# wangzy22/UniPre3D

Measured on AMD Instinct MI355X. Metric: rendered_views_per_sec, higher is better.
Workload: dtype f32; 1 GPU; C2: render-loss hot path (activations + render fwd + loss + render bwd), object-level, P=128 Gaussians/object, 256x256, B=32/GPU x V=4 views = 128 renders/GPU/step; head output o ~ N(0,1) i.i.d. (SURVEY 8d primary regime); global_batch=32, parallelism=dp1, loss=focal_l2, autograd_entry=loss.backward()

## Files before the change

### unipre3d_amd/csrc/u3d_render.hip

```cpp
#include "u3d_common.h"
#ifdef U3D_TIMELINE
#include <cstdio>
#include <vector>
#endif

namespace {

constexpr float LOG2E = 1.4426950408889634f;
constexpr float ALPHA_MIN = 1.0f / 255.0f;
constexpr float T_STOP = 0.0001f;

__device__ __forceinline__ bool rect_hits(const uint2 r, int tx, int ty) {
  const int x0 = r.x & 0xffffu, y0 = r.x >> 16, x1 = r.y & 0xffffu, y1 = r.y >> 16;
  return tx >= x0 && tx < x1 && ty >= y0 && ty < y1;
}

struct LossCtx {
  int kind;
  float w_bg, w_non, b0, b1, b2, t0, t1, t2;
};
__device__ __forceinline__ LossCtx loss_ctx(const U3DLoss& L, const float* __restrict__ bg) {
  const float b0 = bg[0], b1 = bg[1], b2 = bg[2];
  return LossCtx{L.kind, L.w_bg, L.w_non, b0, b1, b2, 1e-6f + 1e-5f * fabsf(b0), 1e-6f + 1e-5f * fabsf(b1), 1e-6f + 1e-5f * fabsf(b2)};
}
// ... 191 lines not shown
        }
      }
#pragma unroll
      for (int k = 0; k < 4; ++k) {
        F.C0[k] = fmaf(Q.z, wv[k], F.C0[k]);
        F.C1[k] = fmaf(Q.w, wv[k], F.C1[k]);
        F.C2[k] = fmaf(R.x, wv[k], F.C2[k]);
        if (DEPTH) F.Dv[k] = fmaf(invd, wv[k], F.Dv[k]);
        F.Tr[k] = tn[k];
      }
      if (contrib != 0ull) { jlast = j; blast = b; }
      if (some_stop) {
#pragma unroll
        for (int k = 0; k < 4; ++k) {
          amin[k] = mask_sel(m_stop[k], 2.f, amin[k]);
          F.stop_pos[k] = __float_as_uint(mask_sel(m_stop[k], R.y, __uint_as_float(F.stop_pos[k])));
        }
        const bool all_done = amin[0] > 1.f && amin[1] > 1.f && amin[2] > 1.f && amin[3] > 1.f;
        if (__ballot(!all_done) == 0ull) { wave_done = true; break; }
      }
    }
    if (blast == b) F.wlast = __builtin_amdgcn_readfirstlane(__float_as_uint(L.P2[jlast].y));
    __builtin_amdgcn_fence(__ATOMIC_RELEASE, "wavefront");
    __builtin_amdgcn_wave_barrier();
  }
  return true;
}

template <typename T>
__device__ __forceinline__ T moment_to_acc(int k, const T* m, float a, float b, float c, float op, float half_w, float half_h) {
  switch (k) {
    case 0: return -(T)half_w * ((T)a * m[0] + (T)b * m[1]);
    case 1: return -(T)half_h * ((T)c * m[1] + (T)b * m[0]);
    case 2: return (T)-0.5 * m[2];
    case 3: return (T)-0.5 * m[3];
    case 4: return (T)-0.5 * m[4];
    case 5: return m[5] != (T)0 ? m[5] / (T)op : (T)0;
    default: return m[k];
  }
}

template <bool HAS_INVD, int PB , bool PLAIN >
__device__ __forceinline__ void tile_backward(const TileLds& L, const TileGeom& G, int lane, uint32_t wmax, int staged,
                                              lanemask_t staged_bal, float pyf, const float (&pxf)[4],
                                              const uint32_t (&lim)[4], float (&Tr)[4], float (&Rk)[4],
                                              const float (&dp0)[4], const float (&dp1)[4], const float (&dp2)[4],
                                              const float (&dinv)[4], float half_w, float half_h, size_t NG,
                                              double* __restrict__ acc, float* __restrict__ pt, uint32_t* __restrict__ pcnt) {
  constexpr int NK = HAS_INVD ? U3D_NACC : U3D_NACC - 1;
  const int bank = (lane >> 2) & 3;
  const bool writer = (lane & 3) == 0 && lane < 16;
  typedef __attribute__((address_space(3))) float lds_float;
  const uint32_t acc_lane = (uint32_t)(uintptr_t)(lds_float*)&L.acc[0][0] + 4u * (uint32_t)bank;
  const int nb = (int)((wmax + U3D_WAVE - 1) / U3D_WAVE);
  for (int b = nb - 1; b >= 0; --b) {
    lanemask_t bal = staged_bal;
    if (b != staged) { bool plain; bal = tile_stage<HAS_INVD>(L, G, lane, b, wmax, plain); staged = b; staged_bal = bal; }
    const uint32_t lm = wmax - (uint32_t)b * U3D_WAVE;
    const int total = lm >= U3D_WAVE ? __popcll(bal) : __popcll(bal & ((1ull << lm) - 1ull));
    for (int j = total - 1; j >= 0; --j) {
      const float4 A = L.P0[j];
      const float4 Q = L.P1[j];
      const float2 R = L.P2[j];
      const float invd = HAS_INVD ? L.D[j] : 0.f;
      const uint32_t pos = __float_as_uint(R.y);
      const float dy = A.y - pyf;
      const float bdy = A.w * dy, cdy2 = (Q.x * dy) * dy;
      float dx[4], ae[4], ar[4];
      lanemask_t any = 0ull;
      if (PLAIN) alpha_run(A.x, A.z, bdy, cdy2, Q.y, L.S[j * L.sstride], pxf[0], ar);
#pragma unroll
      for (int k = 0; k < 4; ++k) {
        dx[k] = A.x - pxf[k];
        float pw = 0.f;
        if (!PLAIN) {
          pw = fmaf(fmaf(A.z, dx[k], bdy), dx[k], cdy2);
          ar[k] = Q.y * __builtin_amdgcn_exp2f(pw);
        }
        const float araw = ar[k];
        const lanemask_t m_a = (PLAIN ? ~0ull : __builtin_amdgcn_fcmpf(pw, 0.f, U3D_FCMP_OLE)) & __builtin_amdgcn_fcmpf(araw, ALPHA_MIN, U3D_FCMP_OGE);
        ae[k] = mask_combine_sel0(m_a, __builtin_amdgcn_uicmp(pos, lim[k], U3D_ICMP_ULT), any, araw);
      }
      if (any == 0ull) continue;
      float m0, mx, mxx, g_r, g_g, g_b, g_d = 0.f;
#pragma unroll
      for (int k = 0; k < 4; ++k) {
        const float alpha = PLAIN ? ae[k] : min_099(ae[k]);
        const float om = 1.f - alpha;
        const float rc = __builtin_amdgcn_rcpf(om);
        const float Tn = Tr[k] * rc;
        const float w = alpha * Tn;
        Tr[k] = Tn;
        float cdp = fmaf(R.x, dp2[k], fmaf(Q.w, dp1[k], Q.z * dp0[k]));
        if (HAS_INVD) cdp = fmaf(invd, dinv[k], cdp);
        const float dL_dalpha = fmaf(Tn, cdp, -(Rk[k] * rc));
        Rk[k] = fmaf(w, cdp, Rk[k]);
        const float q = ae[k] * dL_dalpha;
        const float qdx = q * dx[k];
        if (k == 0) {
          g_r = w * dp0[k]; g_g = w * dp1[k]; g_b = w * dp2[k];
          if (HAS_INVD) g_d = w * dinv[k];
          m0 = q; mx = qdx; mxx = qdx * dx[k];
        } else {
          g_r = fmaf(w, dp0[k], g_r); g_g = fmaf(w, dp1[k], g_g); g_b = fmaf(w, dp2[k], g_b);
          if (HAS_INVD) g_d = fmaf(w, dinv[k], g_d);
          m0 += q; mx += qdx;
          mxx = fmaf(qdx, dx[k], mxx);
        }
      }
      asm volatile("s_nop 1\n\t"
                   "v_add_f32_dpp %0, %0, %0 quad_perm:[1,0,3,2] row_mask:0xf bank_mask:0xf\n\t"
                   "v_add_f32_dpp %1, %1, %1 quad_perm:[1,0,3,2] row_mask:0xf bank_mask:0xf\n\t"
                   "v_add_f32_dpp %2, %2, %2 quad_perm:[1,0,3,2] row_mask:0xf bank_mask:0xf\n\t"
                   "v_add_f32_dpp %3, %3, %3 quad_perm:[1,0,3,2] row_mask:0xf bank_mask:0xf\n\t"
                   "v_add_f32_dpp %4, %4, %4 quad_perm:[1,0,3,2] row_mask:0xf bank_mask:0xf\n\t"
                   "v_add_f32_dpp %5, %5, %5 quad_perm:[1,0,3,2] row_mask:0xf bank_mask:0xf\n\t"
                   "v_add_f32_dpp %0, %0, %0 quad_perm:[2,3,0,1] row_mask:0xf bank_mask:0xf\n\t"
                   "v_add_f32_dpp %1, %1, %1 quad_perm:[2,3,0,1] row_mask:0xf bank_mask:0xf\n\t"
                   "v_add_f32_dpp %2, %2, %2 quad_perm:[2,3,0,1] row_mask:0xf bank_mask:0xf\n\t"
                   "v_add_f32_dpp %3, %3, %3 quad_perm:[2,3,0,1] row_mask:0xf bank_mask:0xf\n\t"
                   "v_add_f32_dpp %4, %4, %4 quad_perm:[2,3,0,1] row_mask:0xf bank_mask:0xf\n\t"
                   "v_add_f32_dpp %5, %5, %5 quad_perm:[2,3,0,1] row_mask:0xf bank_mask:0xf\n\t"
                   "s_nop 1"
                   : "+v"(m0), "+v"(mx), "+v"(mxx), "+v"(g_r), "+v"(g_g), "+v"(g_b));
      if (HAS_INVD)
        asm volatile("s_nop 1\n\t"
                     "v_add_f32_dpp %0, %0, %0 quad_perm:[1,0,3,2] row_mask:0xf bank_mask:0xf\n\t"
                     "s_nop 1\n\t"
                     "v_add_f32_dpp %0, %0, %0 quad_perm:[2,3,0,1] row_mask:0xf bank_mask:0xf\n\t"
                     "s_nop 1"
                     : "+v"(g_d));
      float my = dy * m0, mxy = dy * mx;
      float myy = dy * my;
      if (HAS_INVD)
        asm volatile("s_nop 1\n\t"
                     "v_add_f32_dpp %0, %0, %0 row_half_mirror row_mask:0xf bank_mask:0x5\n\t"
                     "v_add_f32_dpp %1, %1, %1 row_half_mirror row_mask:0xf bank_mask:0x5\n\t"
                     "v_add_f32_dpp %2, %2, %2 row_half_mirror row_mask:0xf bank_mask:0x5\n\t"
                     "v_add_f32_dpp %3, %3, %3 row_half_mirror row_mask:0xf bank_mask:0x5\n\t"
                     "v_add_f32_dpp %4, %4, %4 row_half_mirror row_mask:0xf bank_mask:0x5\n\t"
                     "v_add_f32_dpp %0, %5, %5 row_half_mirror row_mask:0xf bank_mask:0xa\n\t"
                     "v_add_f32_dpp %1, %6, %6 row_half_mirror row_mask:0xf bank_mask:0xa\n\t"
                     "v_add_f32_dpp %2, %7, %7 row_half_mirror row_mask:0xf bank_mask:0xa\n\t"
                     "v_add_f32_dpp %3, %8, %8 row_half_mirror row_mask:0xf bank_mask:0xa\n\t"
                     "v_add_f32_dpp %4, %9, %9 row_half_mirror row_mask:0xf bank_mask:0xa\n\t"
                     "v_add_f32_dpp %0, %0, %0 row_ror:8 row_mask:0xf bank_mask:0x3\n\t"
                     "v_add_f32_dpp %2, %2, %2 row_ror:8 row_mask:0xf bank_mask:0x3\n\t"
                     "v_add_f32_dpp %4, %4, %4 row_ror:8 row_mask:0xf bank_mask:0xf\n\t"
                     "v_add_f32_dpp %0, %1, %1 row_ror:8 row_mask:0xf bank_mask:0xc\n\t"
                     "v_add_f32_dpp %2, %3, %3 row_ror:8 row_mask:0xf bank_mask:0xc\n\t"
                     "s_nop 1"
                     : "+v"(mx), "+v"(mxx), "+v"(myy), "+v"(g_r), "+v"(g_b)
                     : "v"(my), "v"(mxy), "v"(m0), "v"(g_g), "v"(g_d));
      else
        asm volatile("s_nop 1\n\t"
                     "v_add_f32_dpp %0, %0, %0 row_half_mirror row_mask:0xf bank_mask:0x5\n\t"
                     "v_add_f32_dpp %1, %1, %1 row_half_mirror row_mask:0xf bank_mask:0x5\n\t"
                     "v_add_f32_dpp %2, %2, %2 row_half_mirror row_mask:0xf bank_mask:0x5\n\t"
                     "v_add_f32_dpp %3, %3, %3 row_half_mirror row_mask:0xf bank_mask:0x5\n\t"
                     "v_add_f32_dpp %4, %4, %4 row_half_mirror row_mask:0xf bank_mask:0xf\n\t"
                     "v_add_f32_dpp %0, %5, %5 row_half_mirror row_mask:0xf bank_mask:0xa\n\t"
                     "v_add_f32_dpp %1, %6, %6 row_half_mirror row_mask:0xf bank_mask:0xa\n\t"
                     "v_add_f32_dpp %2, %7, %7 row_half_mirror row_mask:0xf bank_mask:0xa\n\t"
                     "v_add_f32_dpp %3, %8, %8 row_half_mirror row_mask:0xf bank_mask:0xa\n\t"
                     "v_add_f32_dpp %4, %4, %4 row_ror:8 row_mask:0xf bank_mask:0xf\n\t"
                     "v_add_f32_dpp %0, %0, %0 row_ror:8 row_mask:0xf bank_mask:0x3\n\t"
                     "v_add_f32_dpp %2, %2, %2 row_ror:8 row_mask:0xf bank_mask:0x3\n\t"
                     "v_add_f32_dpp %0, %1, %1 row_ror:8 row_mask:0xf bank_mask:0xc\n\t"
                     "v_add_f32_dpp %2, %3, %3 row_ror:8 row_mask:0xf bank_mask:0xc\n\t"
                     "s_nop 1"
                     : "+v"(mx), "+v"(mxx), "+v"(myy), "+v"(g_r), "+v"(g_b)
                     : "v"(my), "v"(mxy), "v"(m0), "v"(g_g));
      const uint32_t slot = b < PB ? pos - 1u - (uint32_t)(b * U3D_WAVE) : (uint32_t)j;
      {
        const int xaddr = (lane ^ 32) << 2;
        float t0 = __int_as_float(__builtin_amdgcn_ds_swizzle(__float_as_int(mx), 0x401f));
        float t1 = __int_as_float(__builtin_amdgcn_ds_swizzle(__float_as_int(myy), 0x401f));
        float t2 = __int_as_float(__builtin_amdgcn_ds_swizzle(__float_as_int(g_b), 0x401f));
        mx += t0; myy += t1; g_b += t2;
        t0 = __int_as_float(__builtin_amdgcn_ds_bpermute(xaddr, __float_as_int(mx)));
        t1 = __int_as_float(__builtin_amdgcn_ds_bpermute(xaddr, __float_as_int(myy)));
        t2 = __int_as_float(__builtin_amdgcn_ds_bpermute(xaddr, __float_as_int(g_b)));
        mx += t0; myy += t1; g_b += t2;
      }
      if (writer) {
        lds_float* sl = reinterpret_cast<lds_float*>(acc_lane + __umul24(slot, 40u));
        sl[0] = mx;
        sl[4] = myy;
        if (bank < (HAS_INVD ? 2 : 1)) sl[8] = g_b;
      }
    }
    __builtin_amdgcn_fence(__ATOMIC_RELEASE, "wavefront");
    __builtin_amdgcn_wave_barrier();
    if (b >= PB) {
      if (lane < total) {
        const size_t g = G.vbase + G.sorted_id[G.vbase + __float_as_uint(L.P2[lane].y) - 1u];
        const float4 co = G.conic_op[g];
        float m[U3D_NACC];
#pragma unroll
        for (int k = 0; k < U3D_NACC; ++k) m[k] = L.acc[lane][k];
        bool nz = false;
#pragma unroll
        for (int k = 0; k < NK; ++k) {
          const float v = moment_to_acc<float>(k, m, co.x, co.y, co.z, co.w, half_w, half_h);
          if (v != 0.f) { unsafeAtomicAdd(&acc[(size_t)k * NG + g], (double)v); nz = true; }
        }
        if (nz) {
          G.touched[g] |= U3D_TOUCHED_BIT;
          if (G.tw) u3d_mark_touched_list(G.tw, G.gbase + (g - G.vbase), G.tlist, G.tcount, G.item, (uint32_t)(g - G.vbase));
        }
      }
    } else {
      const uint32_t cnt_b = min(wmax - (uint32_t)b * U3D_WAVE, (uint32_t)U3D_WAVE);
      if ((uint32_t)lane < cnt_b) {
#pragma unroll
        for (int k = 0; k < 5; ++k)
          reinterpret_cast<float2*>(pt + b * (U3D_WAVE * 10))[lane * 5 + k] = reinterpret_cast<const float2*>(&L.acc[lane][0])[k];
      }
    }
    if (b > 0) {
#pragma unroll
      for (int k = 0; k < 5; ++k) reinterpret_cast<float2*>(&L.acc[lane][0])[k] = make_float2(0.f, 0.f);
      __builtin_amdgcn_fence(__ATOMIC_RELEASE, "wavefront");
      __builtin_amdgcn_wave_barrier();
    }
  }
  if (lane == 0) *pcnt = min(wmax, (uint32_t)(PB * U3D_WAVE));
}

__device__ __forceinline__ void load4(const float* __restrict__ p, bool vec, const bool (&inside)[4], float (&v)[4]) {
  v[0] = v[1] = v[2] = v[3] = 0.f;
  if (vec) {
    if (inside[0]) { const float4 t = *reinterpret_cast<const float4*>(p); v[0] = t.x; v[1] = t.y; v[2] = t.z; v[3] = t.w; }
  } else {
#pragma unroll
    for (int k = 0; k < 4; ++k) if (inside[k]) v[k] = p[k];
  }
}
__device__ __forceinline__ void store4(float* __restrict__ p, bool vec, const bool (&inside)[4], const float (&v)[4]) {
  if (vec) {
    if (inside[0]) *reinterpret_cast<float4*>(p) = make_float4(v[0], v[1], v[2], v[3]);
  } else {
#pragma unroll
    for (int k = 0; k < 4; ++k) if (inside[k]) p[k] = v[k];
  }
}

#define U3D_FULL_OCCUPANCY __attribute__((amdgpu_waves_per_eu(7, 7)))
static_assert(TILE_WAVES == 1, "one wave = one workgroup = one tile");
#ifdef U3D_TIMELINE
__device__ uint4* g_timeline = nullptr;
#endif
#define U3D_TILE_PROLOGUE(NWAVES)                                                                       \
  const int lane = threadIdx.x, wave = 0;                                                               \
  uint32_t view_u = blockIdx.y + gridDim.y * blockIdx.z;                                                \
// ... 50 lines not shown
    o0[k] = fmaf(F.Tr[k], bg[0], F.C0[k]); o1[k] = fmaf(F.Tr[k], bg[1], F.C1[k]); o2[k] = fmaf(F.Tr[k], bg[2], F.C2[k]);
    lim[k] = __uint_as_float(F.stop_pos[k]);
  }
  store4(final_T + pid0, vec, inside, F.Tr);
  store4(reinterpret_cast<float*>(n_contrib) + pid0, vec, inside, lim);
  store4(out_color + cid0, vec, inside, o0);
  store4(out_color + cid0 + npix, vec, inside, o1);
  store4(out_color + cid0 + 2 * npix, vec, inside, o2);
  if (DEPTH) store4(out_invdepth + pid0, vec, inside, F.Dv);
  if (lane == 0) tile_last[lid] = F.wlast | (plain ? U3D_TILE_PLAIN_BIT : 0u);
  if (loss.kind != 0) {
    float g0[4], g1[4], g2[4], e = 0.f;
    load4(loss.gt + cid0, vec, inside, g0);
    load4(loss.gt + cid0 + npix, vec, inside, g1);
    load4(loss.gt + cid0 + 2 * npix, vec, inside, g2);
    const LossCtx lc = loss_ctx(loss, bg);
#pragma unroll
    for (int k = 0; k < 4; ++k)
      e += loss_term(lc, loss_weight(lc, inside[k], g0[k], g1[k], g2[k]), o0[k] - g0[k], o1[k] - g1[k], o2[k] - g2[k]);
    e = u3d_wave_sum(e);
    if (lane == 0) loss.partial[lid] = e;
  }
}

#define U3D_BWD_OCCUPANCY __attribute__((amdgpu_waves_per_eu((PB == 1 && !HAS_INVD) ? 7 : 1, (PB == 1 && !HAS_INVD) ? 7 : 10)))
template <bool HAS_INVD, int PB>
__global__ __launch_bounds__(TILE_WAVES * U3D_WAVE) U3D_BWD_OCCUPANCY void render_bwd_wave_kernel(
    U3DSpan span, int H, int W, int tiles_x, int T, uint32_t ntiles_total, uint32_t tile_magic, size_t NG,
    const uint32_t* __restrict__ sorted_id, const uint2* __restrict__ sorted_rect, int rect_indirect, const float2* __restrict__ xy,
    const float4* __restrict__ conic_op, const float4* __restrict__ rgbd, const float* __restrict__ bg,
    const float* __restrict__ dL_dcolor, const float* __restrict__ dL_dinvdepth, const float* __restrict__ final_T,
    const uint32_t* __restrict__ n_contrib, const uint32_t* __restrict__ tile_last, double* __restrict__ acc,
    float* __restrict__ part, const float* __restrict__ out_color, uint32_t* __restrict__ touched, uint32_t* __restrict__ touched_words,
    U3DLoss loss) {
  uint2* const tlist = nullptr;
  uint32_t* const tcount = nullptr;
  __shared__ float4 sP0[TILE_WAVES][U3D_WAVE], sP1[TILE_WAVES][U3D_WAVE];
  __shared__ float2 sP2[TILE_WAVES][U3D_WAVE];
  __shared__ float sD[TILE_WAVES][HAS_INVD ? U3D_WAVE : 1];
  __shared__ __attribute__((aligned(8))) float sAcc[TILE_WAVES][U3D_WAVE][10];
  __shared__ float sS[TILE_WAVES][HAS_INVD ? U3D_WAVE : 1];
  U3D_TILE_PROLOGUE(TILE_WAVES);
  const TileLds L{sP0[wave], sP1[wave], sP2[wave], sD[wave], sAcc[wave], HAS_INVD ? sS[wave] : &sAcc[wave][0][9], HAS_INVD ? 1 : 10};
#pragma unroll
  for (int k = 0; k < 5; ++k) reinterpret_cast<float2*>(&sAcc[wave][lane][0])[k] = make_float2(0.f, 0.f);

  float Tr[4], Rk[4], dp0[4], dp1[4], dp2[4], dinv[4], limf[4];
  uint32_t lim[4];
  load4(final_T + pid0, vec, inside, Tr);
  load4(reinterpret_cast<const float*>(n_contrib) + pid0, vec, inside, limf);
  if (loss.kind != 0) {
    float x0[4], x1[4], x2[4], g0[4], g1[4], g2[4];
    load4(out_color + cid0, vec, inside, x0);
    load4(out_color + cid0 + npix, vec, inside, x1);
    load4(out_color + cid0 + 2 * npix, vec, inside, x2);
    load4(loss.gt + cid0, vec, inside, g0);
    load4(loss.gt + cid0 + npix, vec, inside, g1);
    load4(loss.gt + cid0 + 2 * npix, vec, inside, g2);
    const float sc = loss.dloss[0] * loss.inv_count;
    const LossCtx lc = loss_ctx(loss, bg);
#pragma unroll
    for (int k = 0; k < 4; ++k) {
      dinv[k] = 0.f;
      loss_seed(lc, loss_weight(lc, inside[k], g0[k], g1[k], g2[k]), sc, x0[k] - g0[k], x1[k] - g1[k], x2[k] - g2[k], dp0[k], dp1[k], dp2[k]);
    }
    if (dL_dcolor) {
      float e0[4], e1[4], e2[4];
      load4(dL_dcolor + cid0, vec, inside, e0);
      load4(dL_dcolor + cid0 + npix, vec, inside, e1);
      load4(dL_dcolor + cid0 + 2 * npix, vec, inside, e2);
#pragma unroll
      for (int k = 0; k < 4; ++k) { dp0[k] += e0[k]; dp1[k] += e1[k]; dp2[k] += e2[k]; }
    }
  } else {
    load4(dL_dcolor + cid0, vec, inside, dp0);
    load4(dL_dcolor + cid0 + npix, vec, inside, dp1);
    load4(dL_dcolor + cid0 + 2 * npix, vec, inside, dp2);
    if (HAS_INVD) load4(dL_dinvdepth + pid0, vec, inside, dinv);
    else dinv[0] = dinv[1] = dinv[2] = dinv[3] = 0.f;
  }
#pragma unroll
  for (int k = 0; k < 4; ++k) {
    lim[k] = __float_as_uint(limf[k]);
    Rk[k] = Tr[k] * (bg[0] * dp0[k] + bg[1] * dp1[k] + bg[2] * dp2[k]);
  }
  const uint32_t tl = tile_last[lid];
  if (tl & U3D_TILE_PLAIN_BIT)
    tile_backward<HAS_INVD, PB, true>(L, G, lane, tl & ~U3D_TILE_PLAIN_BIT, -1, 0ull, pyf, pxf, lim, Tr, Rk, dp0, dp1, dp2, dinv, 0.5f * (float)W,
                          0.5f * (float)H, NG, acc, part + (size_t)lid * (PB * U3D_WAVE * 10),
                          reinterpret_cast<uint32_t*>(part + (size_t)ntiles_total * BWD_PART_STRIDE) + lid);
  else
    tile_backward<HAS_INVD, PB, false>(L, G, lane, tl, -1, 0ull, pyf, pxf, lim, Tr, Rk, dp0, dp1, dp2, dinv, 0.5f * (float)W,
                          0.5f * (float)H, NG, acc, part + (size_t)lid * (PB * U3D_WAVE * 10),
                          reinterpret_cast<uint32_t*>(part + (size_t)ntiles_total * BWD_PART_STRIDE) + lid);
}

template <int PB>
__global__ __launch_bounds__(TILE_WAVES * U3D_WAVE) U3D_FULL_OCCUPANCY void render_fb_wave_kernel(
    U3DSpan span, int H, int W, int tiles_x, int T, uint32_t ntiles_total, uint32_t tile_magic, size_t NG,
    const uint32_t* __restrict__ sorted_id, const uint2* __restrict__ sorted_rect, int rect_indirect, const uint32_t* __restrict__ n_vis,
    const float2* __restrict__ xy, const float4* __restrict__ conic_op, const float4* __restrict__ rgbd,
    const float* __restrict__ bg, float* __restrict__ out_color, double* __restrict__ acc, float* __restrict__ part,
    uint32_t* __restrict__ touched, uint32_t* __restrict__ touched_words, uint2* __restrict__ tlist, uint32_t* __restrict__ tcount,
    U3DLoss loss) {
  __shared__ float4 sP0[TILE_WAVES][U3D_WAVE], sP1[TILE_WAVES][U3D_WAVE];
  __shared__ float2 sP2[TILE_WAVES][U3D_WAVE];
  __shared__ __attribute__((aligned(8))) float sAcc[TILE_WAVES][U3D_WAVE][10];
#ifdef U3D_TIMELINE
  const uint64_t tl_t0 = __builtin_amdgcn_s_memrealtime(), tl_c0 = __builtin_amdgcn_s_memtime();
#endif
  U3D_TILE_PROLOGUE(TILE_WAVES);
  const TileLds L{sP0[wave], sP1[wave], sP2[wave], nullptr, sAcc[wave], &sAcc[wave][0][9], 10};
#pragma unroll
  for (int k = 0; k < 5; ++k) reinterpret_cast<float2*>(&sAcc[wave][lane][0])[k] = make_float2(0.f, 0.f);
  TileFwd F;
  const uint32_t nv = n_vis[view];
  const bool plain = tile_forward<false, true>(L, G, lane, nv, pyf, pxf, inside, F);
  if (!plain) tile_forward<false, false>(L, G, lane, nv, pyf, pxf, inside, F);
#ifdef U3D_TIMELINE
  const uint64_t tl_t1 = __builtin_amdgcn_s_memrealtime();
#endif

  float dp0[4], dp1[4], dp2[4], dinv[4], Rk[4], o0[4], o1[4], o2[4], g0[4], g1[4], g2[4];
  float e = 0.f;
#pragma unroll
  for (int k = 0; k < 4; ++k) {
    o0[k] = fmaf(F.Tr[k], bg[0], F.C0[k]); o1[k] = fmaf(F.Tr[k], bg[1], F.C1[k]); o2[k] = fmaf(F.Tr[k], bg[2], F.C2[k]);
  }
  load4(loss.gt + cid0, vec, inside, g0);
  load4(loss.gt + cid0 + npix, vec, inside, g1);
  load4(loss.gt + cid0 + 2 * npix, vec, inside, g2);
  if (out_color) {
    store4(out_color + cid0, vec, inside, o0);
    store4(out_color + cid0 + npix, vec, inside, o1);
    store4(out_color + cid0 + 2 * npix, vec, inside, o2);
  }
  const LossCtx lc = loss_ctx(loss, bg);
#pragma unroll
  for (int k = 0; k < 4; ++k) {
    const float d0 = o0[k] - g0[k], d1 = o1[k] - g1[k], d2 = o2[k] - g2[k];
    const float wk = loss_weight(lc, inside[k], g0[k], g1[k], g2[k]);
    e += loss_term(lc, wk, d0, d1, d2);
    loss_seed(lc, wk, loss.inv_count, d0, d1, d2, dp0[k], dp1[k], dp2[k]);
    dinv[k] = 0.f;
    F.Tr[k] = inside[k] ? F.Tr[k] : 0.f;
    Rk[k] = F.Tr[k] * (bg[0] * dp0[k] + bg[1] * dp1[k] + bg[2] * dp2[k]);
  }
  e = u3d_wave_sum(e);
  if (lane == 0) loss.partial[lid] = e;
#ifdef U3D_TIMELINE
  const uint64_t tl_t2 = __builtin_amdgcn_s_memrealtime();
#endif

  if (plain)
    tile_backward<false, PB, true>(L, G, lane, F.wlast, F.staged, F.staged_bal, pyf, pxf, F.stop_pos, F.Tr, Rk, dp0, dp1, dp2, dinv,
                       0.5f * (float)W, 0.5f * (float)H, NG, acc, part + (size_t)lid * (PB * U3D_WAVE * 10),
                          reinterpret_cast<uint32_t*>(part + (size_t)ntiles_total * BWD_PART_STRIDE) + lid);
  else
    tile_backward<false, PB, false>(L, G, lane, F.wlast, F.staged, F.staged_bal, pyf, pxf, F.stop_pos, F.Tr, Rk, dp0, dp1, dp2, dinv,
                       0.5f * (float)W, 0.5f * (float)H, NG, acc, part + (size_t)lid * (PB * U3D_WAVE * 10),
                          reinterpret_cast<uint32_t*>(part + (size_t)ntiles_total * BWD_PART_STRIDE) + lid);
#ifdef U3D_TIMELINE
  if (lane == 0 && g_timeline) {
    const uint64_t tl_t3 = __builtin_amdgcn_s_memrealtime();
    const uint64_t tl_c1 = __builtin_amdgcn_s_memtime();
    g_timeline[2 * (size_t)lid] = make_uint4((uint32_t)tl_t0, (uint32_t)tl_t3, __builtin_amdgcn_s_getreg((31 << 11) | 4),
                                             (__builtin_amdgcn_s_getreg((31 << 11) | 20) & 15u) | (F.wlast << 4));
    g_timeline[2 * (size_t)lid + 1] = make_uint4((uint32_t)tl_t1, (uint32_t)tl_t2, (uint32_t)(tl_c1 - tl_c0), plain ? 1u : 0u);
  }
#endif
}

constexpr int REDUCE_THREADS = U3D_WAVE * 10;
constexpr int RU = 16, RU1 = 32;
template <int PB>
__global__ __launch_bounds__(REDUCE_THREADS) void bwd_reduce_kernel(U3DSpan span, int T, int NK, int nsplit, size_t NG, float half_w, float half_h,
                                                                   const uint32_t* __restrict__ sorted_id,
                                                                   const float4* __restrict__ conic_op,
                                                                   const float* __restrict__ part,
                                                                   const uint32_t* __restrict__ part_cnt,
                                                                   double* __restrict__ acc, uint32_t* __restrict__ touched,
                                                                   uint32_t* __restrict__ touched_words, int n_loss,
                                                                   const float* __restrict__ loss_partial, float inv_count,
                                                                   float* __restrict__ loss_out, uint2* __restrict__ tlist,
                                                                   uint32_t* __restrict__ tcount, float* __restrict__ zero_fill,
                                                                   size_t zero_floats) {
  __shared__ double s_sum[U3D_WAVE][10];
  __shared__ uint32_t s_cmax;
  if ((int)blockIdx.y > nsplit) {
    const size_t nb = (size_t)gridDim.x * (gridDim.y - nsplit - 1), bid = (size_t)(blockIdx.y - nsplit - 1) * gridDim.x + blockIdx.x;
    const size_t n4 = zero_floats >> 2;
    float4* z4 = reinterpret_cast<float4*>(zero_fill);
    for (size_t e = bid * REDUCE_THREADS + threadIdx.x; e < n4; e += nb * REDUCE_THREADS) z4[e] = make_float4(0.f, 0.f, 0.f, 0.f);
    if (bid == 0 && threadIdx.x < (zero_floats & 3)) zero_fill[(n4 << 2) + threadIdx.x] = 0.f;
    return;
  }
  if ((int)blockIdx.y == nsplit) {
    if (blockIdx.x != 0) return;
    float* sm = reinterpret_cast<float*>(&s_sum[0][0]);
    constexpr int NT = REDUCE_THREADS;
    float a0 = 0.f, a1 = 0.f, a2 = 0.f, a3 = 0.f;
    int i = threadIdx.x;
    for (; i + 3 * NT < n_loss; i += 4 * NT) {
      a0 += loss_partial[i]; a1 += loss_partial[i + NT]; a2 += loss_partial[i + 2 * NT]; a3 += loss_partial[i + 3 * NT];
    }
    for (; i < n_loss; i += NT) a0 += loss_partial[i];
    sm[threadIdx.x] = (a0 + a1) + (a2 + a3);
    __syncthreads();
    if (threadIdx.x < 64) {
      float v = 0.f;
      for (int j = threadIdx.x; j < NT; j += 64) v += sm[j];
#pragma unroll
      for (int o = 32; o > 0; o >>= 1) v += __shfl_xor(v, o);
      if (threadIdx.x == 0) loss_out[0] = v * inv_count;
    }
    return;
  }
  const int view = blockIdx.x, sp = threadIdx.x / 10, k = threadIdx.x - sp * 10;
  const int per = (T + nsplit - 1) / nsplit;
  const int t0 = blockIdx.y * per, t1 = min(T, t0 + per);
  const uint32_t* cnt = part_cnt + (size_t)view * T;
  if (threadIdx.x == 0) s_cmax = 0u;
  __syncthreads();
  {
    uint32_t c = 0u;
    for (int t = t0 + (int)threadIdx.x; t < t1; t += REDUCE_THREADS) c = max(c, cnt[t]);
    if (c != 0u) atomicMax(&s_cmax, c);
  }
  __syncthreads();
  const uint32_t cmax = s_cmax;
  if (cmax == 0u) return;
  constexpr size_t tstride = (size_t)PB * (U3D_WAVE * 10);
#pragma unroll
  for (int h = 0; h < PB; ++h) {
    if (h > 0 && cmax <= (uint32_t)(h * U3D_WAVE)) break;
    const uint32_t spos = (uint32_t)(h * U3D_WAVE + sp);
    double a = 0.0;
    if (k < NK && spos < cmax) {
      const float* base = part + (size_t)view * T * tstride + h * (U3D_WAVE * 10) + threadIdx.x;
      double a0 = 0.0, a1 = 0.0;
      int t = t0;
      for (; t + RU - 1 < t1; t += RU) {
        float v[RU];
        uint32_t c[RU];
#pragma unroll
        for (int u = 0; u < RU; ++u) {
          c[u] = cnt[t + u];
          v[u] = base[(size_t)(t + u) * tstride];
        }
#pragma unroll
        for (int u = 0; u < RU; u += 2) {
          a0 += spos < c[u] ? (double)v[u] : 0.0;
          a1 += spos < c[u + 1] ? (double)v[u + 1] : 0.0;
        }
      }
      for (; t < t1; ++t) {
        const float v0 = base[(size_t)t * tstride];
        a0 += spos < cnt[t] ? (double)v0 : 0.0;
      }
      a = a0 + a1;
    }
    if (h > 0) __syncthreads();
    s_sum[sp][k] = a;
    __syncthreads();
    const bool mine = k < NK && spos < cmax;
    if (h == PB - 1 && !mine) return;
    if (mine) {
      double m[U3D_NACC];
#pragma unroll
      for (int j = 0; j < U3D_NACC; ++j) m[j] = j < NK ? s_sum[sp][j] : 0.0;
      bool any = false;
#pragma unroll
      for (int j = 0; j < U3D_NACC; ++j) any = any || m[j] != 0.0;
      if (any) {
        int Pv;
        size_t vb;
        u3d_view_span(span, view, Pv, vb);
        const size_t g = vb + sorted_id[vb + spos];
        const float4 co = conic_op[g];
        const double outv = moment_to_acc<double>(k, m, co.x, co.y, co.z, co.w, half_w, half_h);
        if (outv != 0.0) unsafeAtomicAdd(&acc[(size_t)k * NG + g], outv);
        if (k == 0) {
          touched[g] |= U3D_TOUCHED_BIT;
          if (touched_words)
            u3d_mark_touched_list(touched_words, u3d_view_gbase(span, view) + (g - vb), tlist, tcount, (uint32_t)(view / span.vpi), (uint32_t)(g - vb));
        }
      }
    }
  }
}

__global__ __launch_bounds__(REDUCE_THREADS) void bwd_reduce1_kernel(U3DSpan span, int T, int NK, int nsplit, size_t NG, float half_w, float half_h,
                                                                   const uint32_t* __restrict__ sorted_id,
                                                                   const float4* __restrict__ conic_op,
                                                                   const float* __restrict__ part,
                                                                   const uint32_t* __restrict__ part_cnt,
                                                                   double* __restrict__ acc, uint32_t* __restrict__ touched,
                                                                   uint32_t* __restrict__ touched_words, int n_loss,
                                                                   const float* __restrict__ loss_partial, float inv_count,
                                                                   float* __restrict__ loss_out) {
  __shared__ double s_sum[U3D_WAVE][10];
  __shared__ uint32_t s_cmax;
  if ((int)blockIdx.y == nsplit) {
    if (blockIdx.x != 0) return;
    float* sm = reinterpret_cast<float*>(&s_sum[0][0]);
    constexpr int NT = REDUCE_THREADS;
    float a0 = 0.f, a1 = 0.f, a2 = 0.f, a3 = 0.f;
    int i = threadIdx.x;
    for (; i + 3 * NT < n_loss; i += 4 * NT) {
      a0 += loss_partial[i]; a1 += loss_partial[i + NT]; a2 += loss_partial[i + 2 * NT]; a3 += loss_partial[i + 3 * NT];
    }
    for (; i < n_loss; i += NT) a0 += loss_partial[i];
    sm[threadIdx.x] = (a0 + a1) + (a2 + a3);
    __syncthreads();
    if (threadIdx.x < 64) {
      float v = 0.f;
      for (int j = threadIdx.x; j < NT; j += 64) v += sm[j];
#pragma unroll
      for (int o = 32; o > 0; o >>= 1) v += __shfl_xor(v, o);
      if (threadIdx.x == 0) loss_out[0] = v * inv_count;
    }
    return;
  }
  const int view = blockIdx.x, sp = threadIdx.x / 10, k = threadIdx.x - sp * 10;
  const int per = (T + nsplit - 1) / nsplit;
  const int t0 = blockIdx.y * per, t1 = min(T, t0 + per);
  const uint32_t* cnt = part_cnt + (size_t)view * T;
  if (threadIdx.x == 0) s_cmax = 0u;
  __syncthreads();
  {
    uint32_t c = 0u;
    for (int t = t0 + (int)threadIdx.x; t < t1; t += REDUCE_THREADS) c = max(c, cnt[t]);
    if (c != 0u) atomicMax(&s_cmax, c);
  }
  __syncthreads();
  const uint32_t cmax = s_cmax;
  if (cmax == 0u) return;
  double a = 0.0;
  if (k < NK && (uint32_t)sp < cmax) {
    const float* base = part + (size_t)view * T * (U3D_WAVE * 10) + threadIdx.x;
    double a0 = 0.0, a1 = 0.0;
    int t = t0;
    for (; t + RU1 - 1 < t1; t += RU1) {
      float v[RU1];
      uint32_t c[RU1];
#pragma unroll
      for (int u = 0; u < RU1; ++u) {
        c[u] = cnt[t + u];
        v[u] = base[(size_t)(t + u) * (U3D_WAVE * 10)];
      }
#pragma unroll
      for (int u = 0; u < RU1; u += 2) {
        a0 += (uint32_t)sp < c[u] ? (double)v[u] : 0.0;
        a1 += (uint32_t)sp < c[u + 1] ? (double)v[u + 1] : 0.0;
      }
    }
    for (; t < t1; ++t) {
      const float v0 = base[(size_t)t * (U3D_WAVE * 10)];
      a0 += (uint32_t)sp < cnt[t] ? (double)v0 : 0.0;
    }
    a = a0 + a1;
  }
  s_sum[sp][k] = a;
  __syncthreads();
  if (k >= NK || (uint32_t)sp >= cmax) return;
  double m[U3D_NACC];
#pragma unroll
  for (int j = 0; j < U3D_NACC; ++j) m[j] = j < NK ? s_sum[sp][j] : 0.0;
  bool any = false;
#pragma unroll
  for (int j = 0; j < U3D_NACC; ++j) any = any || m[j] != 0.0;
  if (!any) return;
  int Pv;
  size_t vb;
  u3d_view_span(span, view, Pv, vb);
  const size_t g = vb + sorted_id[vb + sp];
  const float4 co = conic_op[g];
  const double outv = moment_to_acc<double>(k, m, co.x, co.y, co.z, co.w, half_w, half_h);
  if (outv != 0.0) unsafeAtomicAdd(&acc[(size_t)k * NG + g], outv);
  if (k == 0) {
    touched[g] |= U3D_TOUCHED_BIT;
    if (touched_words) u3d_mark_touched(touched_words, u3d_view_gbase(span, view) + (g - vb));
  }
}


__global__ __launch_bounds__(1024) void loss_reduce_kernel(int n, const float* __restrict__ partial, float inv_count,
                                                           float* __restrict__ loss_out) {
  __shared__ float sm[1024];
  float a0 = 0.f, a1 = 0.f, a2 = 0.f, a3 = 0.f;
  int i = threadIdx.x;
  for (; i + 3072 < n; i += 4096) {
    a0 += partial[i]; a1 += partial[i + 1024]; a2 += partial[i + 2048]; a3 += partial[i + 3072];
  }
  for (; i < n; i += 1024) a0 += partial[i];
  sm[threadIdx.x] = (a0 + a1) + (a2 + a3);
  __syncthreads();
  for (int o = 512; o > 0; o >>= 1) {
    if ((int)threadIdx.x < o) sm[threadIdx.x] += sm[threadIdx.x + o];
    __syncthreads();
  }
  if (threadIdx.x == 0) loss_out[0] = sm[0] * inv_count;
}

}

void u3d_launch_loss_reduce(int n, const float* partial, float inv_count, float* loss_out, hipStream_t s) {
  hipLaunchKernelGGL(loss_reduce_kernel, dim3(1), dim3(1024), 0, s, n, partial, inv_count, loss_out);
}

struct TileGrid { dim3 grid; uint32_t magic; };
static inline TileGrid tile_grid(const u3d_raster_desc& d, int tiles_x, int T) {
  const uint32_t NV = (uint32_t)(d.n_items * d.views_per_item);
  const uint32_t gy = NV < 65535u ? NV : 65535u, gz = (NV + gy - 1u) / gy;
  uint32_t magic = 0u;
  if (tiles_x > 1 && (uint64_t)T * (uint64_t)tiles_x < (1ull << 32)) magic = (uint32_t)(((1ull << 32) + (uint64_t)tiles_x - 1ull) / (uint64_t)tiles_x);
  return TileGrid{dim3((uint32_t)T, gy, gz), magic};
}

void u3d_launch_render_fwd(const u3d_raster_desc& d, const U3DBuffers& b, const float* bg, float* out_color,
                           float* out_invdepth, const U3DLoss& loss, hipStream_t s) {
  const int tiles_x = (d.image_width + U3D_TILE - 1) / U3D_TILE, tiles_y = (d.image_height + U3D_TILE - 1) / U3D_TILE;
  const int T = tiles_x * tiles_y;
  const uint32_t ntiles = (uint32_t)(d.n_items * d.views_per_item * T);
  if (ntiles == 0) return;
  const TileGrid tg = tile_grid(d, tiles_x, T);
  auto* kern = out_invdepth ? render_fwd_wave_kernel<true> : render_fwd_wave_kernel<false>;
  hipLaunchKernelGGL(kern, tg.grid, dim3(TILE_WAVES * U3D_WAVE), 0, s, u3d_span(d), d.image_height, d.image_width,
                     tiles_x, T, ntiles, tg.magic, b.sorted_id, u3d_rect_indirect(d) ? b.rect : b.sorted_rect, u3d_rect_indirect(d), b.n_vis, b.xy, b.conic_op, b.rgbd, bg, out_color,
                     out_invdepth, b.final_T, b.n_contrib, b.tile_last, loss);
}

void u3d_launch_render_fb(const u3d_raster_desc& d, const U3DBuffers& b, const float* bg, float* out_color,
                          const U3DLoss& loss, double* acc, float* part, float* loss_out, hipStream_t s,
                          float* zero_fill, size_t zero_floats, bool list_touched) {
  const int tiles_x = (d.image_width + U3D_TILE - 1) / U3D_TILE, tiles_y = (d.image_height + U3D_TILE - 1) / U3D_TILE;
  const int T = tiles_x * tiles_y;
  const uint32_t ntiles = (uint32_t)(d.n_items * d.views_per_item * T);
  const size_t NG = (size_t)d.views_per_item * u3d_total_P(d);
  if (ntiles == 0 || NG == 0) return;
  const TileGrid tg = tile_grid(d, tiles_x, T);
  uint32_t* tw = u3d_uses_touched_words(d) ? b.touched_words : nullptr;
  uint2* tl = (list_touched && tw) ? b.touched_list : nullptr;
  uint32_t* tc = (list_touched && tw) ? b.touched_count : nullptr;
#ifdef U3D_TIMELINE
  {
    static int launches = 0;
    static uint4* d_tl = nullptr;
    static const char* out = getenv("U3D_TIMELINE_OUT");
    static const int at = getenv("U3D_TIMELINE_AT") ? atoi(getenv("U3D_TIMELINE_AT")) : 150;
    if (out) {
      ++launches;
      if (launches == at) {
        (void)hipMalloc(&d_tl, 2 * sizeof(uint4) * ntiles);
        (void)hipMemset(d_tl, 0, 2 * sizeof(uint4) * ntiles);
        (void)hipMemcpyToSymbol(HIP_SYMBOL(g_timeline), &d_tl, sizeof(d_tl));
      }
      if (launches == at + 6) {
        (void)hipStreamSynchronize(s);
        std::vector<uint4> h(2 * (size_t)ntiles);
        (void)hipMemcpy(h.data(), d_tl, 2 * sizeof(uint4) * ntiles, hipMemcpyDeviceToHost);
        uint4* nul = nullptr;
        (void)hipMemcpyToSymbol(HIP_SYMBOL(g_timeline), &nul, sizeof(nul));
        if (FILE* f = fopen(out, "wb")) { fwrite(h.data(), sizeof(uint4), 2 * (size_t)ntiles, f); fclose(f); }
        fprintf(stderr, "[timeline] %u tiles of launch %d -> %s\n", ntiles, at + 5, out);
      }
    }
  }
#endif
  if (u3d_part_blocks(d) == 1)
    hipLaunchKernelGGL(render_fb_wave_kernel<1>, tg.grid, dim3(TILE_WAVES * U3D_WAVE), 0, s, u3d_span(d), d.image_height, d.image_width,
                       tiles_x, T, ntiles, tg.magic, NG, b.sorted_id, u3d_rect_indirect(d) ? b.rect : b.sorted_rect, u3d_rect_indirect(d), b.n_vis, b.xy, b.conic_op, b.rgbd, bg, out_color,
                       acc, part, b.clamped, tw, tl, tc, loss);
  else
    hipLaunchKernelGGL(render_fb_wave_kernel<U3D_PART_BLOCKS>, tg.grid, dim3(TILE_WAVES * U3D_WAVE), 0, s, u3d_span(d), d.image_height,
                       d.image_width, tiles_x, T, ntiles, tg.magic, NG, b.sorted_id, u3d_rect_indirect(d) ? b.rect : b.sorted_rect, u3d_rect_indirect(d), b.n_vis, b.xy, b.conic_op, b.rgbd, bg,
                       out_color, acc, part, b.clamped, tw, tl, tc, loss);
  const int nsplit = bwd_reduce_split(T, d.n_items * d.views_per_item);
  const int NVi = d.n_items * d.views_per_item;
  if (u3d_part_blocks(d) == 1) {
    hipLaunchKernelGGL(bwd_reduce1_kernel, dim3(NVi, nsplit + 1), dim3(REDUCE_THREADS), 0, s,
                       u3d_span(d), T, U3D_NACC - 1, nsplit, NG, 0.5f * (float)d.image_width, 0.5f * (float)d.image_height, b.sorted_id, b.conic_op, part,
                       reinterpret_cast<const uint32_t*>(part + (size_t)ntiles * BWD_PART_STRIDE), acc, b.clamped, tw, (int)ntiles, loss.partial,
                       loss.inv_count, loss_out);
  } else {
    int zrows = 0;
    if (zero_fill && zero_floats > 0) {
      const size_t want = (zero_floats * sizeof(float) + 65535) / 65536;
      zrows = (int)((want < 256 ? want : 256) + (size_t)NVi - 1) / NVi;
      if (zrows < 1) zrows = 1;
    }
    hipLaunchKernelGGL(bwd_reduce_kernel<U3D_PART_BLOCKS>, dim3(NVi, nsplit + 1 + zrows), dim3(REDUCE_THREADS), 0, s,
                       u3d_span(d), T, U3D_NACC - 1, nsplit, NG, 0.5f * (float)d.image_width, 0.5f * (float)d.image_height, b.sorted_id, b.conic_op, part,
                       reinterpret_cast<const uint32_t*>(part + (size_t)ntiles * BWD_PART_STRIDE), acc, b.clamped, tw, (int)ntiles, loss.partial,
                       loss.inv_count, loss_out, tl, tc, zero_fill, zero_floats);
  }
}

void u3d_launch_render_bwd(const u3d_raster_desc& d, const U3DBuffers& b, const float* bg, const float* dL_dcolor,
                           const float* dL_dinvdepth, const float* out_color, const U3DLoss& loss, double* acc,
                           float* part, hipStream_t s) {
  const int tiles_x = (d.image_width + U3D_TILE - 1) / U3D_TILE, tiles_y = (d.image_height + U3D_TILE - 1) / U3D_TILE;
  const int T = tiles_x * tiles_y;
  const uint32_t ntiles = (uint32_t)(d.n_items * d.views_per_item * T);
  const size_t NG = (size_t)d.views_per_item * u3d_total_P(d);
  if (ntiles == 0 || NG == 0) return;
  const TileGrid tg = tile_grid(d, tiles_x, T);
  const bool invd = dL_dinvdepth && loss.kind == 0;
  uint32_t* tw = u3d_uses_touched_words(d) ? b.touched_words : nullptr;
#define LAUNCH(INVD, PBV)                                                                                                   \
  hipLaunchKernelGGL((render_bwd_wave_kernel<INVD, PBV>), tg.grid, dim3(TILE_WAVES * U3D_WAVE), 0, s, u3d_span(d), d.image_height, \
                     d.image_width, tiles_x, T, ntiles, tg.magic, NG, b.sorted_id, u3d_rect_indirect(d) ? b.rect : b.sorted_rect, u3d_rect_indirect(d), b.xy, b.conic_op, b.rgbd, bg,    \
                     dL_dcolor, dL_dinvdepth, b.final_T, b.n_contrib, b.tile_last, acc, part, out_color, b.clamped, tw, loss)
  if (u3d_part_blocks(d) == 1) { if (invd) LAUNCH(true, 1); else LAUNCH(false, 1); }
  else { if (invd) LAUNCH(true, U3D_PART_BLOCKS); else LAUNCH(false, U3D_PART_BLOCKS); }
#undef LAUNCH
  const int nsplit = bwd_reduce_split(T, d.n_items * d.views_per_item);
  if (u3d_part_blocks(d) == 1)
    hipLaunchKernelGGL(bwd_reduce1_kernel, dim3(d.n_items * d.views_per_item, nsplit), dim3(REDUCE_THREADS), 0, s,
                       u3d_span(d), T, invd ? U3D_NACC : U3D_NACC - 1, nsplit, NG, 0.5f * (float)d.image_width, 0.5f * (float)d.image_height, b.sorted_id,
                       b.conic_op, part, reinterpret_cast<const uint32_t*>(part + (size_t)ntiles * BWD_PART_STRIDE), acc, b.clamped, tw, 0, nullptr, 0.f,
                       nullptr);
  else
    hipLaunchKernelGGL(bwd_reduce_kernel<U3D_PART_BLOCKS>, dim3(d.n_items * d.views_per_item, nsplit), dim3(REDUCE_THREADS), 0, s,
                       u3d_span(d), T, invd ? U3D_NACC : U3D_NACC - 1, nsplit, NG, 0.5f * (float)d.image_width, 0.5f * (float)d.image_height, b.sorted_id,
                       b.conic_op, part, reinterpret_cast<const uint32_t*>(part + (size_t)ntiles * BWD_PART_STRIDE), acc, b.clamped, tw, 0, nullptr, 0.f,
                       nullptr, (uint2*)nullptr, (uint32_t*)nullptr, (float*)nullptr, (size_t)0);
}
```

Measured before the change: 656,400 views/s.

## Reduce per-view backward partials in one block and store results directly

The per-view backward reduction no longer splits tiles across several blocks along grid y. One 1024-thread block per view now splits the tiles across up to four sub-groups sized to the live element count and combines them in shared memory. Because only one block writes each accumulator entry, the double atomic add becomes a plain store. This cuts block count and atomic traffic, but leaves fewer blocks to hide latency and assumes acc needs no prior contribution; cmax is also clamped to the wave size.

```diff
diff --git a/unipre3d_amd/csrc/u3d_render.hip b/unipre3d_amd/csrc/u3d_render.hip
--- a/unipre3d_amd/csrc/u3d_render.hip
+++ b/unipre3d_amd/csrc/u3d_render.hip
@@ -810,28 +810,32 @@
   }
 }
 
-__global__ __launch_bounds__(REDUCE_THREADS) void bwd_reduce1_kernel(U3DSpan span, int T, int NK, int nsplit, size_t NG, float half_w, float half_h,
-                                                                   const uint32_t* __restrict__ sorted_id,
-                                                                   const float4* __restrict__ conic_op,
-                                                                   const float* __restrict__ part,
-                                                                   const uint32_t* __restrict__ part_cnt,
-                                                                   double* __restrict__ acc, uint32_t* __restrict__ touched,
-                                                                   uint32_t* __restrict__ touched_words, int n_loss,
-                                                                   const float* __restrict__ loss_partial, float inv_count,
-                                                                   float* __restrict__ loss_out) {
-  __shared__ double s_sum[U3D_WAVE][10];
+constexpr int RV_THREADS = 1024, RV_SUB = 4;
+__global__ __launch_bounds__(RV_THREADS) void bwd_reduce1_kernel(U3DSpan span, int T, int NK, size_t NG, float half_w, float half_h,
+                                                                 const uint32_t* __restrict__ sorted_id,
+                                                                 const float4* __restrict__ conic_op,
+                                                                 const float* __restrict__ part,
+                                                                 const uint32_t* __restrict__ part_cnt,
+                                                                 double* __restrict__ acc, uint32_t* __restrict__ touched,
+                                                                 uint32_t* __restrict__ touched_words, int n_loss,
+                                                                 const float* __restrict__ loss_partial, float inv_count,
+                                                                 float* __restrict__ loss_out) {
+  __shared__ double s_sum[RV_SUB][U3D_WAVE][10];
   __shared__ uint32_t s_cmax;
-  if ((int)blockIdx.y == nsplit) {
+  if (blockIdx.y == 1) {
     if (blockIdx.x != 0) return;
-    float* sm = reinterpret_cast<float*>(&s_sum[0][0]);
+    float* sm = reinterpret_cast<float*>(&s_sum[0][0][0]);
     constexpr int NT = REDUCE_THREADS;
-    float a0 = 0.f, a1 = 0.f, a2 = 0.f, a3 = 0.f;
-    int i = threadIdx.x;
-    for (; i + 3 * NT < n_loss; i += 4 * NT) {
-      a0 += loss_partial[i]; a1 += loss_partial[i + NT]; a2 += loss_partial[i + 2 * NT]; a3 += loss_partial[i + 3 * NT];
-    }
-    for (; i < n_loss; i += NT) a0 += loss_partial[i];
-    sm[threadIdx.x] = (a0 + a1) + (a2 + a3);
+    static_assert(RV_THREADS >= NT, "the loss row needs REDUCE_THREADS threads");
+    if ((int)threadIdx.x < NT) {
+      float a0 = 0.f, a1 = 0.f, a2 = 0.f, a3 = 0.f;
+      int i = threadIdx.x;
+      for (; i + 3 * NT < n_loss; i += 4 * NT) {
+        a0 += loss_partial[i]; a1 += loss_partial[i + NT]; a2 += loss_partial[i + 2 * NT]; a3 += loss_partial[i + 3 * NT];
+      }
+      for (; i < n_loss; i += NT) a0 += loss_partial[i];
+      sm[threadIdx.x] = (a0 + a1) + (a2 + a3);
+    }
     __syncthreads();
     if (threadIdx.x < 64) {
       float v = 0.f;
@@ -842,51 +846,65 @@
     }
     return;
   }
-  const int view = blockIdx.x, sp = threadIdx.x / 10, k = threadIdx.x - sp * 10;
-  const int per = (T + nsplit - 1) / nsplit;
-  const int t0 = blockIdx.y * per, t1 = min(T, t0 + per);
+  const int view = blockIdx.x;
   const uint32_t* cnt = part_cnt + (size_t)view * T;
   if (threadIdx.x == 0) s_cmax = 0u;
   __syncthreads();
   {
     uint32_t c = 0u;
-    for (int t = t0 + (int)threadIdx.x; t < t1; t += REDUCE_THREADS) c = max(c, cnt[t]);
+    for (int t = threadIdx.x; t < T; t += RV_THREADS) c = max(c, cnt[t]);
     if (c != 0u) atomicMax(&s_cmax, c);
   }
   __syncthreads();
-  const uint32_t cmax = s_cmax;
+  const uint32_t cmax = min(s_cmax, (uint32_t)U3D_WAVE);
   if (cmax == 0u) return;
-  double a = 0.0;
-  if (k < NK && (uint32_t)sp < cmax) {
-    const float* base = part + (size_t)view * T * (U3D_WAVE * 10) + threadIdx.x;
-    double a0 = 0.0, a1 = 0.0;
-    int t = t0;
-    for (; t + RU1 - 1 < t1; t += RU1) {
-      float v[RU1];
-      uint32_t c[RU1];
-#pragma unroll
-      for (int u = 0; u < RU1; ++u) {
-        c[u] = cnt[t + u];
-        v[u] = base[(size_t)(t + u) * (U3D_WAVE * 10)];
-      }
-#pragma unroll
-      for (int u = 0; u < RU1; u += 2) {
-        a0 += (uint32_t)sp < c[u] ? (double)v[u] : 0.0;
-        a1 += (uint32_t)sp < c[u + 1] ? (double)v[u + 1] : 0.0;
-      }
-    }
-    for (; t < t1; ++t) {
-      const float v0 = base[(size_t)t * (U3D_WAVE * 10)];
-      a0 += (uint32_t)sp < cnt[t] ? (double)v0 : 0.0;
-    }
-    a = a0 + a1;
-  }
-  s_sum[sp][k] = a;
+  const int E = (int)cmax * 10, Epad = (E + 63) & ~63;
+  const int S = min(RV_SUB, RV_THREADS / Epad);
+  const int s = threadIdx.x / Epad, e = threadIdx.x - s * Epad;
+  const int sp = e / 10, k = e - sp * 10;
+  const bool live = s < S && e < E;
+  if (live) {
+    double a = 0.0;
+    if (k < NK) {
+      const int per = (T + S - 1) / S;
+      const int t0 = s * per, t1 = min(T, t0 + per);
+      const float* base = part + (size_t)view * T * (U3D_WAVE * 10) + e;
+      double a0 = 0.0, a1 = 0.0;
+      int t = t0;
+      for (; t + RU1 - 1 < t1; t += RU1) {
+        float v[RU1];
+        uint32_t c[RU1];
+#pragma unroll
+        for (int u = 0; u < RU1; ++u) {
+          c[u] = cnt[t + u];
+          v[u] = base[(size_t)(t + u) * (U3D_WAVE * 10)];
+        }
+#pragma unroll
+        for (int u = 0; u < RU1; u += 2) {
+          a0 += (uint32_t)sp < c[u] ? (double)v[u] : 0.0;
+          a1 += (uint32_t)sp < c[u + 1] ? (double)v[u + 1] : 0.0;
+        }
+      }
+      for (; t < t1; ++t) {
+        const float v0 = base[(size_t)t * (U3D_WAVE * 10)];
+        a0 += (uint32_t)sp < cnt[t] ? (double)v0 : 0.0;
+      }
+      a = a0 + a1;
+    }
+    s_sum[s][sp][k] = a;
+  }
   __syncthreads();
-  if (k >= NK || (uint32_t)sp >= cmax) return;
+  if (!live || s != 0 || k >= NK) return;
   double m[U3D_NACC];
 #pragma unroll
-  for (int j = 0; j < U3D_NACC; ++j) m[j] = j < NK ? s_sum[sp][j] : 0.0;
+  for (int j = 0; j < U3D_NACC; ++j) {
+    double v = 0.0;
+    if (j < NK) {
+      v = s_sum[0][sp][j];
+      for (int q = 1; q < S; ++q) v += s_sum[q][sp][j];
+    }
+    m[j] = v;
+  }
   bool any = false;
 #pragma unroll
   for (int j = 0; j < U3D_NACC; ++j) any = any || m[j] != 0.0;
@@ -896,14 +914,12 @@
   u3d_view_span(span, view, Pv, vb);
   const size_t g = vb + sorted_id[vb + sp];
   const float4 co = conic_op[g];
-  const double outv = moment_to_acc<double>(k, m, co.x, co.y, co.z, co.w, half_w, half_h);
-  if (outv != 0.0) unsafeAtomicAdd(&acc[(size_t)k * NG + g], outv);
+  acc[(size_t)k * NG + g] = moment_to_acc<double>(k, m, co.x, co.y, co.z, co.w, half_w, half_h);
   if (k == 0) {
     touched[g] |= U3D_TOUCHED_BIT;
     if (touched_words) u3d_mark_touched(touched_words, u3d_view_gbase(span, view) + (g - vb));
   }
 }
-
 
 __global__ __launch_bounds__(1024) void loss_reduce_kernel(int n, const float* __restrict__ partial, float inv_count,
                                                            float* __restrict__ loss_out) {
@@ -999,8 +1015,8 @@
   const int nsplit = bwd_reduce_split(T, d.n_items * d.views_per_item);
   const int NVi = d.n_items * d.views_per_item;
   if (u3d_part_blocks(d) == 1) {
-    hipLaunchKernelGGL(bwd_reduce1_kernel, dim3(NVi, nsplit + 1), dim3(REDUCE_THREADS), 0, s,
-                       u3d_span(d), T, U3D_NACC - 1, nsplit, NG, 0.5f * (float)d.image_width, 0.5f * (float)d.image_height, b.sorted_id, b.conic_op, part,
+    hipLaunchKernelGGL(bwd_reduce1_kernel, dim3(NVi, 2), dim3(RV_THREADS), 0, s,
+                       u3d_span(d), T, U3D_NACC - 1, NG, 0.5f * (float)d.image_width, 0.5f * (float)d.image_height, b.sorted_id, b.conic_op, part,
                        reinterpret_cast<const uint32_t*>(part + (size_t)ntiles * BWD_PART_STRIDE), acc, b.clamped, tw, (int)ntiles, loss.partial,
                        loss.inv_count, loss_out);
   } else {
@@ -1037,8 +1053,8 @@
 #undef LAUNCH
   const int nsplit = bwd_reduce_split(T, d.n_items * d.views_per_item);
   if (u3d_part_blocks(d) == 1)
-    hipLaunchKernelGGL(bwd_reduce1_kernel, dim3(d.n_items * d.views_per_item, nsplit), dim3(REDUCE_THREADS), 0, s,
-                       u3d_span(d), T, invd ? U3D_NACC : U3D_NACC - 1, nsplit, NG, 0.5f * (float)d.image_width, 0.5f * (float)d.image_height, b.sorted_id,
+    hipLaunchKernelGGL(bwd_reduce1_kernel, dim3(d.n_items * d.views_per_item, 1), dim3(RV_THREADS), 0, s,
+                       u3d_span(d), T, invd ? U3D_NACC : U3D_NACC - 1, NG, 0.5f * (float)d.image_width, 0.5f * (float)d.image_height, b.sorted_id,
                        b.conic_op, part, reinterpret_cast<const uint32_t*>(part + (size_t)ntiles * BWD_PART_STRIDE), acc, b.clamped, tw, 0, nullptr, 0.f,
                        nullptr);
   else
```

Result: slower. 636,000 views/s (-3.1%).

## Normalize backward suffix accumulator and defer quad moment reduction into fused DPP tree

Applied to the files above, without the earlier changes.

Rewrites the backward blending recurrence so the suffix accumulator is stored divided by transmittance. This removes the reciprocal-scaled term and changes the Rk update to a single fma by alpha. The per-pixel x-moments (m0, mx, mxx) are computed in closed form from the four per-lane q values, using the fixed pixel offsets relative to dx[0]. The separate quad-level DPP reduction then shrinks to three values folded after the half-row mirror pass, cutting DPP instructions per Gaussian. Numerical behaviour changes slightly, and the closed form assumes a fixed 4-pixel spacing along x.

```diff
diff --git a/unipre3d_amd/csrc/u3d_render.hip b/unipre3d_amd/csrc/u3d_render.hip
--- a/unipre3d_amd/csrc/u3d_render.hip
+++ b/unipre3d_amd/csrc/u3d_render.hip
@@ -297,7 +297,7 @@
         ae[k] = mask_combine_sel0(m_a, __builtin_amdgcn_uicmp(pos, lim[k], U3D_ICMP_ULT), any, araw);
       }
       if (any == 0ull) continue;
-      float m0, mx, mxx, g_r, g_g, g_b, g_d = 0.f;
+      float m0, mx, mxx, g_r, g_g, g_b, g_d = 0.f, q[4];
 #pragma unroll
       for (int k = 0; k < 4; ++k) {
         const float alpha = PLAIN ? ae[k] : min_099(ae[k]);
@@ -308,43 +308,26 @@
         Tr[k] = Tn;
         float cdp = fmaf(R.x, dp2[k], fmaf(Q.w, dp1[k], Q.z * dp0[k]));
         if (HAS_INVD) cdp = fmaf(invd, dinv[k], cdp);
-        const float dL_dalpha = fmaf(Tn, cdp, -(Rk[k] * rc));
-        Rk[k] = fmaf(w, cdp, Rk[k]);
-        const float q = ae[k] * dL_dalpha;
-        const float qdx = q * dx[k];
+        const float dl = cdp - Rk[k];
+        Rk[k] = fmaf(alpha, dl, Rk[k]);
+        q[k] = PLAIN ? w * dl : ae[k] * (Tn * dl);
         if (k == 0) {
           g_r = w * dp0[k]; g_g = w * dp1[k]; g_b = w * dp2[k];
           if (HAS_INVD) g_d = w * dinv[k];
-          m0 = q; mx = qdx; mxx = qdx * dx[k];
         } else {
           g_r = fmaf(w, dp0[k], g_r); g_g = fmaf(w, dp1[k], g_g); g_b = fmaf(w, dp2[k], g_b);
           if (HAS_INVD) g_d = fmaf(w, dinv[k], g_d);
-          m0 += q; mx += qdx;
-          mxx = fmaf(qdx, dx[k], mxx);
         }
       }
-      asm volatile("s_nop 1\n\t"
-                   "v_add_f32_dpp %0, %0, %0 quad_perm:[1,0,3,2] row_mask:0xf bank_mask:0xf\n\t"
-                   "v_add_f32_dpp %1, %1, %1 quad_perm:[1,0,3,2] row_mask:0xf bank_mask:0xf\n\t"
-                   "v_add_f32_dpp %2, %2, %2 quad_perm:[1,0,3,2] row_mask:0xf bank_mask:0xf\n\t"
-                   "v_add_f32_dpp %3, %3, %3 quad_perm:[1,0,3,2] row_mask:0xf bank_mask:0xf\n\t"
-                   "v_add_f32_dpp %4, %4, %4 quad_perm:[1,0,3,2] row_mask:0xf bank_mask:0xf\n\t"
-                   "v_add_f32_dpp %5, %5, %5 quad_perm:[1,0,3,2] row_mask:0xf bank_mask:0xf\n\t"
-                   "v_add_f32_dpp %0, %0, %0 quad_perm:[2,3,0,1] row_mask:0xf bank_mask:0xf\n\t"
-                   "v_add_f32_dpp %1, %1, %1 quad_perm:[2,3,0,1] row_mask:0xf bank_mask:0xf\n\t"
-                   "v_add_f32_dpp %2, %2, %2 quad_perm:[2,3,0,1] row_mask:0xf bank_mask:0xf\n\t"
-                   "v_add_f32_dpp %3, %3, %3 quad_perm:[2,3,0,1] row_mask:0xf bank_mask:0xf\n\t"
-                   "v_add_f32_dpp %4, %4, %4 quad_perm:[2,3,0,1] row_mask:0xf bank_mask:0xf\n\t"
-                   "v_add_f32_dpp %5, %5, %5 quad_perm:[2,3,0,1] row_mask:0xf bank_mask:0xf\n\t"
-                   "s_nop 1"
-                   : "+v"(m0), "+v"(mx), "+v"(mxx), "+v"(g_r), "+v"(g_g), "+v"(g_b));
-      if (HAS_INVD)
-        asm volatile("s_nop 1\n\t"
-                     "v_add_f32_dpp %0, %0, %0 quad_perm:[1,0,3,2] row_mask:0xf bank_mask:0xf\n\t"
-                     "s_nop 1\n\t"
-                     "v_add_f32_dpp %0, %0, %0 quad_perm:[2,3,0,1] row_mask:0xf bank_mask:0xf\n\t"
-                     "s_nop 1"
-                     : "+v"(g_d));
+      {
+        const float dc = dx[0] - 1.5f;
+        const float s03 = q[0] + q[3], s12 = q[1] + q[2];
+        const float t1 = fmaf(1.5f, q[3] - q[0], 0.5f * (q[2] - q[1]));
+        const float t2 = fmaf(2.25f, s03, 0.25f * s12);
+        m0 = s03 + s12;
+        mx = fmaf(dc, m0, -t1);
+        mxx = fmaf(dc, mx - t1, t2);
+      }
       float my = dy * m0, mxy = dy * mx;
       float myy = dy * my;
       if (HAS_INVD)
@@ -386,6 +369,15 @@
                      "s_nop 1"
                      : "+v"(mx), "+v"(mxx), "+v"(myy), "+v"(g_r), "+v"(g_b)
                      : "v"(my), "v"(mxy), "v"(m0), "v"(g_g));
+      asm volatile("s_nop 1\n\t"
+                   "v_add_f32_dpp %0, %0, %0 quad_perm:[1,0,3,2] row_mask:0xf bank_mask:0xf\n\t"
+                   "v_add_f32_dpp %1, %1, %1 quad_perm:[1,0,3,2] row_mask:0xf bank_mask:0xf\n\t"
+                   "v_add_f32_dpp %2, %2, %2 quad_perm:[1,0,3,2] row_mask:0xf bank_mask:0xf\n\t"
+                   "v_add_f32_dpp %0, %0, %0 quad_perm:[2,3,0,1] row_mask:0xf bank_mask:0xf\n\t"
+                   "v_add_f32_dpp %1, %1, %1 quad_perm:[2,3,0,1] row_mask:0xf bank_mask:0xf\n\t"
+                   "v_add_f32_dpp %2, %2, %2 quad_perm:[2,3,0,1] row_mask:0xf bank_mask:0xf\n\t"
+                   "s_nop 1"
+                   : "+v"(mx), "+v"(myy), "+v"(g_b));
       const uint32_t slot = b < PB ? pos - 1u - (uint32_t)(b * U3D_WAVE) : (uint32_t)j;
       {
         const int xaddr = (lane ^ 32) << 2;
@@ -602,7 +594,7 @@
 #pragma unroll
   for (int k = 0; k < 4; ++k) {
     lim[k] = __float_as_uint(limf[k]);
-    Rk[k] = Tr[k] * (bg[0] * dp0[k] + bg[1] * dp1[k] + bg[2] * dp2[k]);
+    Rk[k] = bg[0] * dp0[k] + bg[1] * dp1[k] + bg[2] * dp2[k];
   }
   const uint32_t tl = tile_last[lid];
   if (tl & U3D_TILE_PLAIN_BIT)
@@ -664,7 +656,7 @@
     loss_seed(lc, wk, loss.inv_count, d0, d1, d2, dp0[k], dp1[k], dp2[k]);
     dinv[k] = 0.f;
     F.Tr[k] = inside[k] ? F.Tr[k] : 0.f;
-    Rk[k] = F.Tr[k] * (bg[0] * dp0[k] + bg[1] * dp1[k] + bg[2] * dp2[k]);
+    Rk[k] = bg[0] * dp0[k] + bg[1] * dp1[k] + bg[2] * dp2[k];
   }
   e = u3d_wave_sum(e);
   if (lane == 0) loss.partial[lid] = e;
```

New measurement: 656,800 views/s before, 690,100 views/s after, median of 6. +5.1%, better.
